# USTC-Computer-Vision/tracking

Measured on AMD Instinct MI355X. Metric: MixtureOfGaussianV2BGS throughput (Mpixels/s; concurrent 1080p30 streams in streams_1080p30), higher is better.
Workload: dtype f32

## Files before the change

tracking_amd/csrc/engine_mog2.h:

```cpp

int mog2_check(bgs_algo, const bgs_params& p) {
  if (p.mog2_nmixtures != bgs::kMog2K) return fail(BGS_ERR_UNSUPPORTED, "MOG2 kernel is built for K=%d mixtures, got %d", bgs::kMog2K, p.mog2_nmixtures);
  return BGS_OK;
}

int mog2_check_geometry(bgs_algo, int, int, int ch) {
  if (ch != 3) return fail(BGS_ERR_UNSUPPORTED, "MixtureOfGaussianV2BGS needs 3 channels: getBackgroundImage asserts nchannels == 3 (MixtureOfGaussianV2BGS.cpp:59)");
  return BGS_OK;
}

struct Mog2State : FamilyState {
  DevPtr<uint8_t> model;
  int sparse_now = 2;
  int sparse_want = 2;
  unsigned launches = 0;
  unsigned confirmed4 = 0;
  unsigned every_left = 0;
  unsigned filter_launches = 0;
  DevPtr<unsigned> d_stat;
  static constexpr int kStatSlots = 8;
  unsigned* h_stat = nullptr;
  hipEvent_t stat_ev[kStatSlots] = {nullptr};
  bool stat_posted[kStatSlots] = {false};
  unsigned stat_seq = 0;
  ~Mog2State() override {
    model.reset(), d_stat.reset();
    if (h_stat) (void)hipHostFree(h_stat);
    for (hipEvent_t ev : stat_ev)
      if (ev) (void)hipEventDestroy(ev);
  }
};
Mog2State& mog2_of(const bgs_engine* e) { return state_of<Mog2State>(e); }

void mog2_stat_read(Mog2State& st) {
  int slot = -1;
  for (unsigned back = 1; back <= (unsigned)Mog2State::kStatSlots && back <= st.stat_seq; ++back) {
    const int i = (int)((st.stat_seq - back) % Mog2State::kStatSlots);
    if (!st.stat_posted[i]) break;
    if (slot < 0 && hipEventQuery(st.stat_ev[i]) == hipSuccess) slot = i;
    if (slot >= 0) st.stat_posted[i] = false;
  }
  if (slot < 0) return;
  const unsigned* hs = st.h_stat + 3 * slot;
  const unsigned total = hs[0], live = hs[1], need = hs[2];
  if (total < 64 * 5) return;
  const float lf = (float)live / (float)total, nf = (float)need / (float)total;
  const int want = (nf < 0.5f * lf && lf - nf > 0.1f) ? 4 : lf < 0.7f ? 2 : 1;
  const bool clear = (want == 4 && nf < 0.35f * lf) || (want != 4 && st.sparse_now == 4 && nf > 0.8f * lf);
  static const bool debug = getenv("BGS_DEBUG_STAT") != nullptr;
  if (debug)
    fprintf(stderr, "[bgs] mog2 auto: %u record slots sampled, %.3f live, %.3f needed after the summaries -> mode %d (now %d)\n", total, lf, nf, want, st.sparse_now);
  const bool confirms = want == 4 && st.sparse_now == 4;
  if (want != st.sparse_now && (clear || want == st.sparse_want)) st.sparse_now = want;
  st.sparse_want = want;
  if (confirms) {
    st.confirmed4++;
  } else {
    st.confirmed4 = 0;
    st.every_left = 8;
  }
}
void mog2_stat_post(Mog2State& st, hipStream_t s) {
  const int i = (int)(st.stat_seq % Mog2State::kStatSlots);
  (void)hipMemcpyAsync(st.h_stat + 3 * i, st.d_stat, 3 * sizeof(unsigned), hipMemcpyDeviceToHost, s);
  (void)hipMemsetAsync(st.d_stat, 0, 3 * sizeof(unsigned), s);
  (void)hipEventRecord(st.stat_ev[i], s);
  st.stat_posted[i] = true;
  st.stat_seq++;
}

int launch_mog2(bgs_engine* e, bgs::Mog2Args& a, hipStream_t s, bool timed = true) {
  const bgs_params& p = e->p;
  a.shadow = p.mog2_detect_shadows && (!p.enable_threshold || ((p.mog2_shadow_value > p.threshold) != (255 > p.threshold)));
  a.want_bg = a.bgimg != nullptr, a.packed = a.fg_bits != nullptr;
  a.xcd_swizzle = e->knob.xcd_swizzle, a.complete = e->knob.mog2_complete;
  Mog2State& st = mog2_of(e);
  const bool autom = timed && e->knob.mog2_sparse == 3;
  if (autom) mog2_stat_read(st);
  int mode = e->knob.mog2_sparse == 3 ? st.sparse_now : e->knob.mog2_sparse;
  const bool every_mean = a.shadow || a.want_bg;
  if (mode >= 4 && every_mean) mode = 2;
  bool sample = false;
  if (autom && mode != 4) {
    const unsigned n = st.launches++;
    if ((n & (n < 64 ? 3u : 15u)) == 0) sample = true, mode = every_mean ? 2 : 4;
  } else if (autom) {
    if (st.every_left > 0 || st.confirmed4 < 2) {
      sample = true;
      if (st.every_left > 0) st.every_left--;
    } else {
      sample = (st.filter_launches++ & 7u) == 0;
    }
  }
  if (mode >= 4 && every_mean) return fail(BGS_ERR_INVALID, "MOG2: the filter kernel cannot deliver the shadow test or the background image");
  a.sparse = mode;
  a.stat = sample ? st.d_stat.p : nullptr;
  if (a.packed && a.npix % 64) return fail(BGS_ERR_UNSUPPORTED, "packed mask needs pixels %% 64 == 0");
  Timed t(e, s, "mog2_update_kernel", timed);
  const dim3 grid(blocks_for(a.npix)), block(bgs::kBlock);
  unsigned every = 1;
  while (grid.x / every > 256) every <<= 1;
  a.stat_mask = every - 1;
  if (mode >= 4)
    hipLaunchKernelGGL((bgs::mog2_update_kernel<bgs::kMog2Filter>), grid, block, 0, s, a);
  else if (mode >= 2)
    hipLaunchKernelGGL((bgs::mog2_update_kernel<bgs::kMog2Count>), grid, block, 0, s, a);
  else
    hipLaunchKernelGGL((bgs::mog2_update_kernel<bgs::kMog2Eager>), grid, block, 0, s, a);
  if (a.stat) mog2_stat_post(st, s);
  return BGS_OK;
}

void mog2_fill_args(const bgs_engine* e, bgs::Mog2Args& m, double lr) {
  const bgs_params& p = e->p;
  m.state = mog2_of(e).model;
  m.alphaT = (float)lr, m.alpha1 = 1.f - m.alphaT, m.prune = (float)(-lr * (double)p.mog2_ct);
  m.Tb = p.mog2_var_threshold, m.TB = p.mog2_background_ratio, m.Tg = p.mog2_var_threshold_gen;
  m.s_min = bgs::mog2_smin(bgs::mog2_tq(m.Tb > m.Tg ? m.Tb : m.Tg));
  m.varInit = p.mog2_var_init, m.varMin = p.mog2_var_min, m.varMax = p.mog2_var_max, m.tau = p.mog2_tau;
  m.thr = p.threshold, m.enable_thr = p.enable_threshold, m.shadow_val = p.mog2_shadow_value;
}

void mog2_clear(bgs_engine* e, const bgs::Mog2Args& m, hipStream_t s) {
  hipLaunchKernelGGL(bgs::mog2_clear_kernel, dim3(blocks_for(m.npix)), dim3(bgs::kBlock), 0, s, m);
}

int launch_mog2_clip(bgs_engine* e, bgs::Mog2ClipArgs& c, int fuse, hipStream_t s) {
  const bgs_params& p = e->p;
  bgs::Mog2Args& a = c.m;
  a.shadow = p.mog2_detect_shadows && (!p.enable_threshold || ((p.mog2_shadow_value > p.threshold) != (255 > p.threshold)));
  a.want_bg = a.bgimg != nullptr, a.packed = a.fg_bits != nullptr;
  a.xcd_swizzle = e->knob.xcd_swizzle, a.complete = e->knob.mog2_complete;
  a.sparse = e->knob.mog2_sparse == 0 ? 0 : 1;
  a.stat = nullptr;
  if (a.packed && a.npix % 64) return fail(BGS_ERR_UNSUPPORTED, "packed mask needs pixels %% 64 == 0");
  Timed t(e, s, "mog2_clip_kernel");
  const dim3 grid(blocks_for(a.npix)), block(bgs::kBlock);
  unsigned every = 1;
  while (grid.x / every > 256) every <<= 1;
  a.stat_mask = every - 1;
#define MOG2_CLIP_CASE(TV) \
  if (fuse == TV) hipLaunchKernelGGL((bgs::mog2_clip_kernel<TV>), grid, block, 0, s, c);
  MOG2_CLIP_CASE(2) MOG2_CLIP_CASE(4) MOG2_CLIP_CASE(8)
#undef MOG2_CLIP_CASE
  return BGS_OK;
}

size_t mog2_state_bytes(const bgs_engine* e) {
  const size_t P = e->n * e->S;
  return (P + bgs::kMog2Tile - 1) / bgs::kMog2Tile * bgs::kMog2TileBytes;
}

int mog2_allocate(bgs_engine* e) {
  Mog2State& st = make_state<Mog2State>(e);
  HIP_TRY(hipMalloc((void**)&st.d_stat.p, 3 * sizeof(unsigned)));
  HIP_TRY(hipMemsetAsync(st.d_stat, 0, 3 * sizeof(unsigned), e->stream()));
  HIP_TRY(hipHostMalloc((void**)&st.h_stat, 3 * Mog2State::kStatSlots * sizeof(unsigned), hipHostMallocDefault));
  for (hipEvent_t& ev : st.stat_ev) HIP_TRY(hipEventCreateWithFlags(&ev, hipEventDisableTiming));
  return model_allocate(e, st.model, mog2_state_bytes(e));
}

uint64_t mog2_key(const bgs_engine* e, int i) { return mog_lr_key(e, i, e->p.mog2_history, 2); }

int mog2_run(bgs_engine* e, int first, int count, const uint8_t* d_frames, uint8_t* d_fg, uint8_t* d_bg, uint64_t* d_bits, hipStream_t s, uint32_t* flags) {
  const bgs_params& p = e->p;
  double lr = p.alpha;
  int64_t nframes = e->seen[first];
  bgs::Mog2Args m{};
  m.state_off = e->n * first, m.npix = e->n * count;
  mog2_fill_args(e, m, 0.0);
  if (nframes == 0 || lr >= 1) {
    mog2_clear(e, m, s);
    nframes = 0;
  }
  ++nframes;
  const int64_t n2 = 2 * nframes;
  lr = (lr >= 0 && nframes > 1) ? lr : 1. / (double)std::min<int64_t>(n2, p.mog2_history);
  mog2_fill_args(e, m, lr);
  m.frame = d_frames, m.fg = d_fg, m.bgimg = d_bg, m.fg_bits = d_bits;
  int rc = launch_mog2(e, m, s);
  if (rc) return rc;
  if (nframes == 1)
    for (int i = first; i < first + count; ++i) e->seen[i] = 0;
  *flags = BGS_FG_VALID | BGS_BG_VALID;
  return BGS_OK;
}

int mog2_clip_fused(bgs_engine* e, int first, int count, int fuse, size_t slab, const uint8_t* fr, uint8_t* fg, uint8_t* bg, uint64_t* bits, hipStream_t s, uint32_t* flags) {
  const bgs_params& p = e->p;
  const int64_t seen = e->seen[first];
  bgs::Mog2ClipArgs c{};
  c.m.state_off = e->n * first, c.m.npix = e->n * count;
  mog2_fill_args(e, c.m, 0.0);
  if (seen == 0) mog2_clear(e, c.m, s);
  for (int j = 0; j < fuse; ++j) {
    const int64_t nf = seen + j + 1;
    const double lr = (p.alpha >= 0 && nf > 1) ? p.alpha : 1. / (double)std::min<int64_t>(2 * nf, p.mog2_history);
    c.alphaT[j] = (float)lr, c.alpha1[j] = 1.f - c.alphaT[j], c.prune[j] = (float)(-lr * (double)p.mog2_ct);
  }
  c.m.frame = fr, c.m.fg = fg, c.m.bgimg = bg, c.m.fg_bits = bits;
  c.frame_stride = slab * 3, c.fg_stride = slab, c.bg_stride = slab * 3, c.bits_stride = slab / 64;
  *flags = BGS_FG_VALID | BGS_BG_VALID;
  return launch_mog2_clip(e, c, fuse, s);
}

int64_t mog2_get_state(bgs_engine* e, int stream, const char* plane, void* dst, size_t cap) {
  const size_t n = e->n, off = n * stream;
  int p0 = -1, np = 0;
  if (!strcmp(plane, "w")) p0 = 0, np = 5;
  if (!strcmp(plane, "var")) p0 = 5, np = 5;
  if (!strcmp(plane, "mu")) p0 = 10, np = 15;
  if (!strcmp(plane, "summary")) p0 = 100, np = 5;
  const bool nm = !strcmp(plane, "nmodes") || !strcmp(plane, "summary_valid");
  const bool want_valid = !strcmp(plane, "summary_valid");
  if (p0 < 0 && !nm) return unknown_plane(e, plane);
  const size_t need = nm ? n : (size_t)np * n * 4;
  if (cap < need) return too_small(plane);
  const size_t T = bgs::kMog2Tile, TB = bgs::kMog2TileBytes;
  const size_t t0 = off / T, t1 = (off + n + T - 1) / T;
  std::vector<uint8_t> tiles((t1 - t0) * TB);
  if (fetch(tiles.data(), mog2_of(e).model + t0 * TB, tiles.size())) return BGS_ERR_HIP;
  for (size_t i = 0; i < n; ++i) {
    const size_t sp = off + i, in = sp % T;
    const uint8_t* tb = tiles.data() + (sp / T - t0) * TB;
    const float* w = reinterpret_cast<const float*>(tb) + in;
    const float* rec = reinterpret_cast<const float*>(tb + bgs::kMog2RecOff) + in * 4;
    const uint16_t* sum = reinterpret_cast<const uint16_t*>(tb + bgs::kMog2SumOff) + in;
    const unsigned meta = reinterpret_cast<const uint16_t*>(tb + bgs::kMog2MetaOff)[in];
    if (nm) {
      ((uint8_t*)dst)[i] = want_valid ? (uint8_t)((meta >> 15) & 1u) : (uint8_t)bgs::mog2_meta_count(meta);
      continue;
    }
    for (int r = 0; r < bgs::kMog2K; ++r) {
      const unsigned f = (meta >> (3 * r)) & 7u;
      const float* rc = f ? rec + (size_t)(f - 1) * T * 4 : nullptr;
      if (p0 == 100) ((uint32_t*)dst)[(size_t)r * n + i] = f ? sum[(size_t)(f - 1) * T] : 0u;
      if (p0 == 0) ((float*)dst)[(size_t)r * n + i] = f ? w[(size_t)r * T] : 0.f;
      if (p0 == 5) ((float*)dst)[(size_t)r * n + i] = f ? rc[0] : 0.f;
      if (p0 == 10)
        for (int c = 0; c < 3; ++c) ((float*)dst)[((size_t)r * 3 + c) * n + i] = f ? rc[1 + c] : 0.f;
    }
  }
  return (int64_t)need;
}

constexpr Family kMog2 = [] {
  Family f{};
  f.check = mog2_check, f.check_geometry = mog2_check_geometry, f.allocate = mog2_allocate, f.key = mog2_key, f.run = mog2_run;
  f.get_state = mog2_get_state, f.clip_fused = mog2_clip_fused, f.clip_fusable = mog_clip_fusable;
  return f;
}();
```

tracking_amd/csrc/kernel_mog2.h:

```cpp
#pragma once
#include "bgs_device.h"

namespace bgs {

constexpr int kMog2K = 5;
constexpr int kMog2Tile = 256;
constexpr size_t kMog2TileBytes = (size_t)kMog2Tile * (4 * kMog2K + 2 * kMog2K + 16 * kMog2K + 2);
constexpr size_t kMog2SumOff = (size_t)kMog2Tile * 4 * kMog2K;
constexpr size_t kMog2RecOff = kMog2SumOff + (size_t)kMog2Tile * 2 * kMog2K;
constexpr size_t kMog2MetaOff = kMog2RecOff + (size_t)kMog2Tile * 16 * kMog2K;
static_assert(kMog2Tile % 64 == 0, "a wave that starts on a multiple of 64 pixels stays inside one tile, any other touches at most two");

struct Mog2Args {
  const uint8_t* frame;
  uint8_t* fg;
  uint8_t* bgimg;
  uint64_t* fg_bits;
  uint8_t* state;
  size_t state_off;
  size_t npix;
  float alphaT, alpha1, prune;
  float Tb, TB, Tg, varInit, varMin, varMax, tau;
  int thr, enable_thr, shadow_val;
  int shadow, want_bg, packed;
  unsigned* stat;
  unsigned stat_mask;
  int sparse;
  int complete;
  int xcd_swizzle;
  uint32_t s_min;
};

struct Mog2Ptr {
  float* w;
  uint16_t* sum;
  float4* rec;
  uint16_t* meta;
};
__device__ __forceinline__ Mog2Ptr mog2_ptr(uint8_t* state, size_t sp) {
  uint8_t* tb = state + (sp / kMog2Tile) * kMog2TileBytes;
  const size_t in = sp % kMog2Tile;
  Mog2Ptr p;
  p.w = reinterpret_cast<float*>(tb) + in;
  p.sum = reinterpret_cast<uint16_t*>(tb + kMog2SumOff) + in;
  p.rec = reinterpret_cast<float4*>(tb + kMog2RecOff) + in;
  p.meta = reinterpret_cast<uint16_t*>(tb + kMog2MetaOff) + in;
  return p;
}
__device__ __forceinline__ size_t mog2_uniform(size_t v) {
  asm("" : "+s"(v));
  return v;
}
struct Mog2Lane {
  uint8_t* state;
  size_t bw, bs, br, bm;
  uint32_t o4, o2, o16;
  static constexpr int kMid = 2 * 4 * kMog2Tile;
  __device__ __forceinline__ float* w(int r) const { return reinterpret_cast<float*>(state + bw + (size_t)o4 + (r * 4 * kMog2Tile - kMid)); }
  __device__ __forceinline__ uint16_t* sum(int s) const { return reinterpret_cast<uint16_t*>(state + bs + (size_t)o2 + s * 2 * kMog2Tile); }
  __device__ __forceinline__ float4* rec(int s) const { return reinterpret_cast<float4*>(state + mog2_uniform(br + (size_t)s * 16 * kMog2Tile) + (size_t)o16); }
  __device__ __forceinline__ float* w_of(uint32_t r) const { return reinterpret_cast<float*>(state + mog2_uniform(bw - kMid) + (size_t)(o4 + r * (4u * kMog2Tile))); }
  __device__ __forceinline__ float4* rec_of(uint32_t s) const { return reinterpret_cast<float4*>(state + br + (size_t)(o16 + s * (16u * kMog2Tile))); }
  __device__ __forceinline__ uint16_t* meta() const { return reinterpret_cast<uint16_t*>(state + bm + (size_t)o2); }
};
__device__ __forceinline__ Mog2Lane mog2_lane(uint8_t* state, size_t first, uint32_t lane) {
  Mog2Lane l;
  const size_t tb = (first / kMog2Tile) * kMog2TileBytes;
  l.state = state;
  l.bw = mog2_uniform(tb + Mog2Lane::kMid), l.bs = mog2_uniform(tb + kMog2SumOff), l.br = mog2_uniform(tb + kMog2RecOff), l.bm = mog2_uniform(tb + kMog2MetaOff);
  const uint32_t in0 = (uint32_t)(first % kMog2Tile);
  uint32_t in = in0 + lane, skip = 0;
  if (in0 + (kWave - 1) >= (uint32_t)kMog2Tile) {
    const bool next = in >= (uint32_t)kMog2Tile;
    in = next ? in - kMog2Tile : in;
    skip = next ? (uint32_t)kMog2TileBytes : 0u;
  }
  l.o4 = in * 4 + skip, l.o2 = in * 2 + skip, l.o16 = in * 16 + skip;
  return l;
}
__device__ __host__ __forceinline__ int mog2_meta_count(unsigned meta) {
  unsigned t = (meta | (meta >> 1) | (meta >> 2)) & 0x1249u;
#ifdef __HIP_DEVICE_COMPILE__
  return __popc(t);
#else
  t = (t & 1u) + ((t >> 3) & 1u) + ((t >> 6) & 1u) + ((t >> 9) & 1u) + ((t >> 12) & 1u);
  return (int)t;
#endif
}

constexpr float kMog2SumVar = 32.f, kMog2SumVarTight = 24.f;
__device__ __host__ __forceinline__ uint32_t mog2_summary(float var, float m0, float m1, float m2) {
  const bool inside = m0 >= 0.f && m0 < 256.f && m1 >= 0.f && m1 < 256.f && m2 >= 0.f && m2 < 256.f;
  const uint32_t cls = (inside && var <= kMog2SumVarTight) ? 0u : 1u;
  const uint32_t q0 = inside ? (uint32_t)(int)m0 >> 3 : 0u, q1 = inside ? (uint32_t)(int)m1 >> 3 : 0u, q2 = inside ? (uint32_t)(int)m2 >> 3 : 0u;
  return q0 | (q1 << 5) | (q2 << 10) | (cls << 15);
}
__device__ __host__ __forceinline__ bool mog2_summary_ok(uint32_t word, float var, float m0, float m1, float m2) {
  const float b0 = (float)((word & 0x1fu) << 3), b1 = (float)(((word >> 5) & 0x1fu) << 3), b2 = (float)(((word >> 10) & 0x1fu) << 3);
  const float e0 = m0 - b0, e1 = m1 - b1, e2 = m2 - b2;
  const bool means = (e0 >= -2.f && e0 <= 9.f) && (e1 >= -2.f && e1 <= 9.f) && (e2 >= -2.f && e2 <= 9.f);
  const bool tightable = var <= kMog2SumVarTight && m0 >= 0.f && m0 < 256.f && m1 >= 0.f && m1 < 256.f && m2 >= 0.f && m2 < 256.f;
  return (word >> 15) ? !tightable : (means && var <= kMog2SumVar);
}
__device__ __host__ __forceinline__ uint32_t mog2_tq(float Tmax) {
  const float c = 3.f * kMog2SumVar * Tmax;
  return c < 1.0e9f ? (uint32_t)(int)c + 4u : 0xffffffffu;
}
constexpr uint32_t kMog2SMax = 93u, kMog2SNever = 0xffffffffu;
__device__ __host__ __forceinline__ uint32_t mog2_smin(uint32_t tq) {
  for (uint32_t S = 4u; S <= kMog2SMax; ++S) {
    const uint32_t B = 8u * S - 28u;
    if (B * B > tq) return S;
  }
  return kMog2SNever;
}
__device__ __host__ __forceinline__ uint32_t mog2_pixq(uint32_t pix) { return (pix >> 3) & 0x1f1f1fu; }
__device__ __host__ __forceinline__ uint32_t mog2_spread(uint32_t word) { return (word & 0x1fu) | ((word << 3) & 0x1f00u) | ((word << 6) & 0x1f0000u); }
__device__ __host__ __forceinline__ bool mog2_reject_s(uint32_t word, uint32_t S, uint32_t s_min) { return !(word >> 15) & (S >= s_min); }
__device__ __forceinline__ bool mog2_reject(uint32_t word, uint32_t pixq, uint32_t s_min) {
  return mog2_reject_s(word, __builtin_amdgcn_sad_u8(pixq, mog2_spread(word), 0u), s_min);
}

enum { kMog2Stream = 0, kMog2BySlot = 1, kMog2Ranked = 2, kMog2One = 3 };
struct Mog2Px {
  float w[kMog2K];
  int sl[kMog2K];
};
struct Mog2Recs {
  float4 rc[kMog2K];
  int k0, cnt;
  unsigned cm, bgm, mm;
};

template <int ORD>
__device__ __forceinline__ void mog2_swap(Mog2Px& s, Mog2Recs& R, int i, int j) {
  const float t = s.w[i];
  s.w[i] = s.w[j], s.w[j] = t;
  const int u = s.sl[i];
  s.sl[i] = s.sl[j], s.sl[j] = u;
  if constexpr (ORD == kMog2Ranked) {
    const float4 c = R.rc[i];
    R.rc[i] = R.rc[j], R.rc[j] = c;
  }
}

template <int ORD>
__device__ __forceinline__ float4 mog2_pick(const Mog2Recs& R, int code) {
  static_assert(ORD == kMog2BySlot, "ranked records are indexed by rank; the filter kernel holds one record or none");
  float4 v = make_float4(0.f, 0.f, 0.f, 0.f);
#pragma unroll
  for (int j = 0; j < kMog2K; ++j) {
    const bool here = code == j + 1;
    const float4 c = R.rc[j];
    v.x = here ? c.x : v.x, v.y = here ? c.y : v.y, v.z = here ? c.z : v.z, v.w = here ? c.w : v.w;
  }
  return v;
}
template <int ORD>
__device__ __forceinline__ float4 mog2_rec_at(const Mog2Px& s, const Mog2Recs& R, int mode) {
  if constexpr (ORD == kMog2Ranked)
    return R.rc[mode];
  else
    return mog2_pick<ORD>(R, s.sl[mode]);
}
template <int ORD>
__device__ __forceinline__ float4 mog2_pick_now(const Mog2Recs& R, int code, int hit, float4 out) {
  const float4 v = mog2_pick<ORD>(R, code);
  const bool h = code == hit;
  return make_float4(h ? out.x : v.x, h ? out.y : v.y, h ? out.z : v.z, h ? out.w : v.w);
}

template <int ORD>
__device__ __forceinline__ float4 mog2_rec_now(const Mog2Px& s, const Mog2Recs& R, int mode, int hit, float4 out) {
  if constexpr (ORD == kMog2Ranked)
    return R.rc[mode];
  else
    return mog2_pick_now<ORD>(R, s.sl[mode], hit, out);
}

template <int ORD>
__device__ __forceinline__ bool mog2_shadow(const Mog2Px& s, const Mog2Recs& R, int hit, float4 out, int nmodes, float x0, float x1, float x2, const Mog2Args& a) {
  bool done = false, result = false;
  float tWeight = 0.f;
#pragma unroll
  for (int mode = 0; mode < kMog2K; ++mode) {
    if (mode < nmodes && !done) {
      const float4 v = mog2_rec_now<ORD>(s, R, mode, hit, out);
      float num = 0.0f, den = 0.0f;
      num += x0 * v.y;
      den += v.y * v.y;
      num += x1 * v.z;
      den += v.z * v.z;
      num += x2 * v.w;
      den += v.w * v.w;
      if (den == 0) {
        done = true;
      } else {
        if (num <= den && num >= a.tau * den) {
          const float q = div_rn(num, den);
          float d2a = 0.0f, dD;
          dD = q * v.y - x0, d2a += dD * dD;
          dD = q * v.z - x1, d2a += dD * dD;
          dD = q * v.w - x2, d2a += dD * dD;
          if (d2a < a.Tb * v.x * q * q) result = true, done = true;
        }
        if (!done) {
          tWeight += s.w[mode];
          if (tWeight > a.TB) done = true;
        }
      }
    }
  }
  return result;
}

template <int ORD>
__device__ __forceinline__ int mog2_pixel(Mog2Px& s, Mog2Recs& R, int& nmodes_io, float x0, float x1, float x2, const Mog2Args& a, int& hit, float4& out,
                                          const float alphaT, const float alpha1, const float prune, const unsigned rej) {
  bool background = false, fitsPDF = false;
  int nmodes = nmodes_io;
  const int nNewModes = nmodes;
  float totalWeight = 0.f;
  hit = 0;
  out = make_float4(0.f, 0.f, 0.f, 0.f);
#pragma unroll
  for (int mode = 0; mode < kMog2K; ++mode) {
    if (mode < nmodes) {
      float weight = alpha1 * s.w[mode] + prune;
      bool matched = false;
      if (!fitsPDF && !((rej >> s.sl[mode]) & 1u)) {
        const float4 v = mog2_rec_at<ORD>(s, R, mode);
        const float var = v.x;
        const float d0 = v.y - x0, d1 = v.z - x1, d2 = v.w - x2;
        const float dist2 = d0 * d0 + d1 * d1 + d2 * d2;
        if (totalWeight < a.TB && dist2 < a.Tb * var) background = true;
        if (dist2 < a.Tg * var) {
          fitsPDF = true;
          matched = true;
          weight += alphaT;
          const float k = div_rn(alphaT, weight);
          float varnew = var + k * (dist2 - var);
          varnew = varnew > a.varMin ? varnew : a.varMin;
          varnew = varnew < a.varMax ? varnew : a.varMax;
          out = make_float4(varnew, v.y - k * d0, v.z - k * d1, v.w - k * d2);
          hit = s.sl[mode];
          if constexpr (ORD == kMog2Ranked) R.rc[mode] = out;
        }
      }
      const bool pruned = weight < -prune;
      if (pruned) nmodes--;
      s.w[mode] = pruned ? 0.f : weight;
      if (matched) {
        bool moving = true;
#pragma unroll
        for (int i = mode; i > 0; --i) {
          moving = moving && !(weight < s.w[i - 1]);
          if (moving) mog2_swap<ORD>(s, R, i, i - 1);
        }
      }
      totalWeight += pruned ? 0.f : weight;
    }
  }
  totalWeight = div_rn(1.f, totalWeight);
#pragma unroll
  for (int mode = 0; mode < kMog2K; ++mode)
    if (mode < nmodes) s.w[mode] *= totalWeight;
  nmodes = nNewModes;
  if (!fitsPDF) {
    const int slot = (nmodes == kMog2K) ? s.sl[kMog2K - 1] : nmodes + 1;
    const int mode = (nmodes == kMog2K) ? kMog2K - 1 : nmodes++;
#pragma unroll
    for (int k = 0; k < kMog2K; ++k) {
      if (k == mode) {
        s.w[k] = (nmodes == 1) ? 1.f : alphaT;
        s.sl[k] = slot;
        if constexpr (ORD == kMog2Ranked) R.rc[k] = make_float4(a.varInit, x0, x1, x2);
      } else if (nmodes != 1 && k < nmodes - 1) {
        s.w[k] *= alpha1;
      }
    }
    out = make_float4(a.varInit, x0, x1, x2);
    hit = slot;
    bool moving = true;
#pragma unroll
    for (int i = kMog2K - 1; i > 0; --i) {
      if (i <= nmodes - 1) {
        moving = moving && !(alphaT < s.w[i - 1]);
        if (moving) mog2_swap<ORD>(s, R, i, i - 1);
      }
    }
  }
  nmodes_io = nmodes;
  if (background) return 0;
  if (a.shadow) {
    if (mog2_shadow<ORD>(s, R, hit, out, nmodes, x0, x1, x2, a)) return a.shadow_val;
  }
  return 255;
}

template <int ORD, bool FEAT>
__device__ __forceinline__ int mog2_pixel_lockstep(Mog2Px& s, const Mog2Recs& R, const Mog2Lane& mp, const int wave_cand, int& nmodes_io, float x0, float x1,
                                                   float x2, const Mog2Args& a, int& hit, float4& out, const float alphaT, const float alpha1, const float prune) {
  static_assert(ORD != kMog2Ranked, "records by slot, streamed, or the single one");
  static_assert(!FEAT || ORD == kMog2BySlot, "the shadow test needs every record in registers");
  bool background = false, fitsPDF = false;
  int nmodes = nmodes_io;
  const int nNewModes = nmodes;
  float totalWeight = 0.f;
  hit = 0;
  out = make_float4(0.f, 0.f, 0.f, 0.f);
  unsigned cm = 0, bgm = 0, mm = 0;
  bool c1 = false, b1 = false, m1 = false;
  int k1 = 0;
  if constexpr (ORD == kMog2One) {
    const float4 v = R.rc[0];
    const float d0 = v.y - x0, d1 = v.z - x1, d2 = v.w - x2;
    const float dist2 = d0 * d0 + d1 * d1 + d2 * d2;
    c1 = R.cnt > 0, k1 = R.k0 + 1;
    b1 = dist2 < a.Tb * v.x, m1 = dist2 < a.Tg * v.x;
  } else if constexpr (ORD == kMog2Stream) {
    cm = R.cm, bgm = R.bgm, mm = R.mm;
  } else {
#pragma unroll
    for (int j = 0; j < kMog2K; ++j) {
      if (j < wave_cand) {
        const float4 v = R.rc[j];
        const float d0 = v.y - x0, d1 = v.z - x1, d2 = v.w - x2;
        const float dist2 = d0 * d0 + d1 * d1 + d2 * d2;
        const int code = j + 1;
        const bool is = j < R.cnt;
        cm |= (unsigned)is << code;
        bgm |= (unsigned)(is && dist2 < a.Tb * v.x) << code;
        mm |= (unsigned)(is && dist2 < a.Tg * v.x) << code;
      }
    }
  }
  float wmatch = 0.f;
  int rstar = 0;
#pragma unroll
  for (int mode = 0; mode < kMog2K; ++mode) {
    if (mode < nmodes) {
      float weight = alpha1 * s.w[mode] + prune;
      const int code = s.sl[mode];
      const bool c = ORD == kMog2One ? (c1 && code == k1) : (bool)((cm >> code) & 1u);
      if (!fitsPDF && c) {
        const bool b = ORD == kMog2One ? b1 : (bool)((bgm >> code) & 1u);
        const bool m = ORD == kMog2One ? m1 : (bool)((mm >> code) & 1u);
        if (totalWeight < a.TB && b) background = true;
        if (m) {
          fitsPDF = true;
          weight += alphaT;
          wmatch = weight, rstar = mode, hit = code;
        }
      }
      const bool pruned = weight < -prune;
      if (pruned) nmodes--;
      s.w[mode] = pruned ? 0.f : weight;
      totalWeight += pruned ? 0.f : weight;
    }
  }
  if (fitsPDF) {
    float4 v;
    if constexpr (ORD == kMog2Stream)
      v = *mp.rec_of((uint32_t)(hit - 1));
    else if constexpr (ORD == kMog2One)
      v = R.rc[0];
    else
      v = wave_cand == 1 ? R.rc[0] : mog2_pick<ORD>(R, hit);
    const float var = v.x;
    const float d0 = v.y - x0, d1 = v.z - x1, d2 = v.w - x2;
    const float dist2 = d0 * d0 + d1 * d1 + d2 * d2;
    const float k = div_rn(alphaT, wmatch);
    float varnew = var + k * (dist2 - var);
    varnew = varnew > a.varMin ? varnew : a.varMin;
    varnew = varnew < a.varMax ? varnew : a.varMax;
    out = make_float4(varnew, v.y - k * d0, v.z - k * d1, v.w - k * d2);
    bool moving = true;
#pragma unroll
    for (int i = kMog2K - 1; i > 0; --i) {
      const bool in = i <= rstar;
      moving = in ? (moving & !(wmatch < s.w[i - 1])) : moving;
      const bool sw = in & moving;
      const float wi = s.w[i], wj = s.w[i - 1];
      s.w[i] = sw ? wj : wi, s.w[i - 1] = sw ? wi : wj;
      const int ci = s.sl[i], cj = s.sl[i - 1];
      s.sl[i] = sw ? cj : ci, s.sl[i - 1] = sw ? ci : cj;
    }
  }
  totalWeight = div_rn(1.f, totalWeight);
#pragma unroll
  for (int mode = 0; mode < kMog2K; ++mode)
    if (mode < nmodes) s.w[mode] *= totalWeight;
  nmodes = nNewModes;
  if (!fitsPDF) {
    const int slot = (nmodes == kMog2K) ? s.sl[kMog2K - 1] : nmodes + 1;
    const int mode = (nmodes == kMog2K) ? kMog2K - 1 : nmodes++;
#pragma unroll
    for (int k = 0; k < kMog2K; ++k) {
      if (k == mode) {
        s.w[k] = (nmodes == 1) ? 1.f : alphaT;
        s.sl[k] = slot;
      } else if (nmodes != 1 && k < nmodes - 1) {
        s.w[k] *= alpha1;
      }
    }
    out = make_float4(a.varInit, x0, x1, x2);
    hit = slot;
    bool moving = true;
    Mog2Recs none;
#pragma unroll
    for (int i = kMog2K - 1; i > 0; --i) {
      if (i <= nmodes - 1) {
        moving = moving && !(alphaT < s.w[i - 1]);
        if (moving) mog2_swap<ORD>(s, none, i, i - 1);
      }
    }
  }
  nmodes_io = nmodes;
  if (background) return 0;
  if constexpr (FEAT) {
    if (a.shadow) {
      if (mog2_shadow<ORD>(s, R, hit, out, nmodes, x0, x1, x2, a)) return a.shadow_val;
    }
  }
  return 255;
}

template <int ORD>
__device__ __forceinline__ void mog2_background(const Mog2Px& s, const Mog2Recs& R, int hit, float4 out, int nmodes, float TB, int& b0, int& b1, int& b2) {
  float v0 = 0.f, v1 = 0.f, v2 = 0.f, totalWeight = 0.f;
  bool stop = false;
#pragma unroll
  for (int g = 0; g < kMog2K; ++g) {
    if (g < nmodes && !stop) {
      const float4 v = mog2_rec_now<ORD>(s, R, g, hit, out);
      const float w = s.w[g];
      v0 += w * v.y;
      v1 += w * v.z;
      v2 += w * v.w;
      totalWeight += w;
      if (totalWeight > TB) stop = true;
    }
  }
  const float inv = div_rn(1.f, totalWeight);
  b0 = sat_u8(v0 * inv), b1 = sat_u8(v1 * inv), b2 = sat_u8(v2 * inv);
}

__device__ __forceinline__ void mog2_group_or(unsigned v, unsigned& or2, unsigned& or8, unsigned& or16) {
  v |= (unsigned)__builtin_amdgcn_mov_dpp((int)v, 0xB1, 0xf, 0xf, true);
  or2 = v;
  v |= (unsigned)__builtin_amdgcn_mov_dpp((int)v, 0x4E, 0xf, 0xf, true);
  v |= (unsigned)__builtin_amdgcn_mov_dpp((int)v, 0x141, 0xf, 0xf, true);
  or8 = v;
  v |= (unsigned)__builtin_amdgcn_mov_dpp((int)v, 0x140, 0xf, 0xf, true);
  or16 = v;
}

__device__ __forceinline__ void mog2_stream(const Mog2Lane& mp, Mog2Recs& R, const unsigned need, const bool valid_in, const bool sampled, const uint32_t pix,
                                            const Mog2Args& a, uint32_t (&sm)[kMog2K], int& would) {
  const float x0 = (float)(pix & 0xffu), x1 = (float)((pix >> 8) & 0xffu), x2 = (float)(pix >> 16);
  const uint32_t pixq = mog2_pixq(pix), k_first = (uint32_t)R.k0;
  const bool rebuild = __any(!valid_in);
  unsigned cm = 0, bgm = 0, mm = 0;
  int fresh = 0;
  float4 cur = *mp.rec_of((need & 1u) ? 0u : k_first);
#pragma unroll
  for (int k = 0; k < kMog2K; ++k) {
    float4 nxt = cur;
    if (k + 1 < kMog2K) nxt = *mp.rec_of(((need >> (k + 1)) & 1u) ? (uint32_t)(k + 1) : k_first);
    const bool is = (need >> k) & 1u;
    const float d0 = cur.y - x0, d1 = cur.z - x1, d2 = cur.w - x2;
    const float dist2 = d0 * d0 + d1 * d1 + d2 * d2;
    cm |= (unsigned)is << (k + 1);
    bgm |= (unsigned)(is && dist2 < a.Tb * cur.x) << (k + 1);
    mm |= (unsigned)(is && dist2 < a.Tg * cur.x) << (k + 1);
    if (rebuild) {
      const uint32_t word = mog2_summary(cur.x, cur.y, cur.z, cur.w);
      const bool mine = is && !valid_in;
      sm[k] = mine ? word : sm[k];
      if (sampled) fresh += (int)(mine && !mog2_reject(word, pixq, a.s_min));
    }
    cur = nxt;
  }
  R.cm = cm, R.bgm = bgm, R.mm = mm;
  would = valid_in ? would : fresh;
}

__device__ __forceinline__ void mog2_stat_add(const Mog2Args& a, const uint32_t lane, const int nm_in, const int would) {
  unsigned s_live = 0, s_need = 0;
#pragma unroll
  for (int bit = 0; bit < 3; ++bit) {
    s_live += (unsigned)__popcll(__ballot((nm_in >> bit) & 1)) << bit;
    s_need += (unsigned)__popcll(__ballot((would >> bit) & 1)) << bit;
  }
  const unsigned lanes = (unsigned)__popcll(__ballot(1));
  if (lane == 0) {
    atomicAdd(a.stat, lanes * kMog2K);
    atomicAdd(a.stat + 1, s_live);
    atomicAdd(a.stat + 2, s_need);
  }
}

constexpr int kMog2ClipMax = 8;
struct Mog2ClipArgs {
  Mog2Args m;
  size_t frame_stride;
  size_t fg_stride, bg_stride, bits_stride;
  float alphaT[kMog2ClipMax], alpha1[kMog2ClipMax], prune[kMog2ClipMax];
};

enum { kMog2Eager = 1, kMog2Count = 2, kMog2Filter = 4 };

template <int MODE, int T>
__device__ __forceinline__ void mog2_body(const Mog2Args& a, const size_t frame_stride, const size_t fg_stride, const size_t bg_stride, const size_t bits_stride,
                                          const float* alphaT, const float* alpha1, const float* prune) {
  static_assert(T == 1 || MODE == kMog2Eager, "clip launches load eagerly");
  constexpr int ORD = MODE == kMog2Filter ? kMog2Stream : T > 1 ? kMog2Ranked : kMog2BySlot;
  constexpr bool FEAT = MODE != kMog2Filter;
  size_t blk = blockIdx.x;
  if (a.xcd_swizzle) {
    const size_t per = gridDim.x >> 3, main = per << 3;
    if (blk < main) blk = (blk & 7) * per + (blk >> 3);
  }
  const uint32_t lane = threadIdx.x & (kWave - 1);
  const size_t pw = blk * kBlock + (uint32_t)__builtin_amdgcn_readfirstlane((int)(threadIdx.x & ~(uint32_t)(kWave - 1)));
  if (pw >= a.npix) return;
  const size_t left = a.npix - pw;
  if (lane >= (left < (size_t)kWave ? (uint32_t)left : (uint32_t)kWave)) return;
  uint32_t pix[T];
  const uint8_t* const fw = a.frame + pw * 3;
#pragma unroll
  for (int t = 0; t < T; ++t) {
    const uint8_t* f = fw + (size_t)t * frame_stride + lane * 3u;
    pix[t] = (uint32_t)f[0] | ((uint32_t)f[1] << 8) | ((uint32_t)f[2] << 16);
  }
  const Mog2Lane mp = mog2_lane(a.state, a.state_off + pw, lane);
  const unsigned meta_raw = *mp.meta();
  const unsigned meta_in = meta_raw & 0x7fffu;
  const bool valid_in = (meta_raw >> 15) & 1u;
  const int nm_in = mog2_meta_count(meta_in);
  const bool dense = MODE == kMog2Eager && a.sparse == 0;
  const bool sampled = MODE != kMog2Eager && a.stat && (blockIdx.x & a.stat_mask) == 0;
  float wv[kMog2K];
  uint32_t sm[kMog2K];
  Mog2Recs R;
  R.cnt = kMog2K;
  int wave_cand = kMog2K;
#pragma unroll
  for (int k = 0; k < kMog2K; ++k) sm[k] = 0u;
  if constexpr (MODE == kMog2Eager) {
#pragma unroll
    for (int k = 0; k < kMog2K; ++k) {
      wv[k] = *mp.w(k);
      R.rc[k] = *mp.rec(k);
      if (dense) sm[k] = *mp.sum(k);
    }
  } else if constexpr (MODE == kMog2Count) {
    wv[0] = *mp.w(0);
    R.rc[0] = *mp.rec(0);
    int wave_nm = 0;
#pragma unroll
    for (int n = 1; n <= kMog2K; ++n)
      if (__any(nm_in >= n)) wave_nm = n;
    wave_cand = wave_nm <= 2 ? 2 : wave_nm;
    if (wave_nm <= 2) {
      const uint32_t idx = 1 < nm_in ? 1u : 0u;
      wv[1] = *mp.w_of(idx), R.rc[1] = *mp.rec_of(idx);
#pragma unroll
      for (int k = 2; k < kMog2K; ++k) wv[k] = 0.f, R.rc[k] = make_float4(0.f, 0.f, 0.f, 0.f);
    } else {
#pragma unroll
      for (int k = 1; k < kMog2K; ++k) {
        const uint32_t idx = k < nm_in ? (uint32_t)k : 0u;
        wv[k] = *mp.w_of(idx), R.rc[k] = *mp.rec_of(idx);
      }
    }
#pragma unroll
    for (int k = 0; k < kMog2K; ++k) wv[k] = k < nm_in ? wv[k] : 0.f;
    R.cnt = nm_in;
  } else {
#pragma unroll
    for (int k = 0; k < kMog2K; ++k) wv[k] = *mp.w(k), sm[k] = *mp.sum(k);
    const uint32_t pixq = mog2_pixq(pix[0]);
    unsigned need = 0;
#pragma unroll
    for (int k = 0; k < kMog2K; ++k) {
      const bool live = k < nm_in;
      const bool r = (live & valid_in) & mog2_reject(sm[k], pixq, a.s_min);
      need |= (unsigned)(live && !r) << k;
    }
    R.cnt = __popc(need);
    R.k0 = (int)min((unsigned)__builtin_ctzg(need, 32), (unsigned)(kMog2K - 1));
    int would = R.cnt;
    if (!__any(R.cnt > 1)) {
      wave_cand = 1;
      R.rc[0] = *mp.rec_of((uint32_t)R.k0);
      if (sampled && !valid_in) {
        const float4 c = R.rc[0];
        would = (int)(R.cnt > 0 && !mog2_reject(mog2_summary(c.x, c.y, c.z, c.w), pixq, a.s_min));
      }
    } else {
      mog2_stream(mp, R, need, valid_in, sampled, pix[0], a, sm, would);
    }
    if (sampled) mog2_stat_add(a, lane, nm_in, would);
  }
  if constexpr (MODE == kMog2Count) {
    if (sampled) mog2_stat_add(a, lane, nm_in, nm_in);
  }
  Mog2Px s;
#pragma unroll
  for (int r = 0; r < kMog2K; ++r) s.sl[r] = (int)((meta_in >> (3 * r)) & 7u), s.w[r] = wv[r];
  if constexpr (ORD == kMog2Ranked) {
    Mog2Recs Q;
#pragma unroll
    for (int r = 0; r < kMog2K; ++r) Q.rc[r] = mog2_pick<kMog2BySlot>(R, s.sl[r]);
#pragma unroll
    for (int r = 0; r < kMog2K; ++r) R.rc[r] = Q.rc[r];
  }
  unsigned dirty = 0;
  const bool one = MODE == kMog2Filter && wave_cand == 1;
  int nm = nm_in, hit = 0;
  float4 out = make_float4(0.f, 0.f, 0.f, 0.f);
#pragma unroll
  for (int t = 0; t < T; ++t) {
    const float x0 = (float)(pix[t] & 0xffu), x1 = (float)((pix[t] >> 8) & 0xffu), x2 = (float)(pix[t] >> 16);
    int raw;
    if constexpr (ORD == kMog2Ranked)
      raw = mog2_pixel<ORD>(s, R, nm, x0, x1, x2, a, hit, out, alphaT[t], alpha1[t], prune[t], 0u);
    else if (one)
      raw = mog2_pixel_lockstep<kMog2One, false>(s, R, mp, 1, nm, x0, x1, x2, a, hit, out, alphaT[t], alpha1[t], prune[t]);
    else
      raw = mog2_pixel_lockstep<ORD, FEAT>(s, R, mp, wave_cand, nm, x0, x1, x2, a, hit, out, alphaT[t], alpha1[t], prune[t]);
    const int m = thr_bin(raw, a.thr, a.enable_thr);
    if (a.fg) (a.fg + pw + (size_t)t * fg_stride)[lane] = (uint8_t)m;
    if (a.packed) {
      const uint64_t word = __ballot(m != 0);
      if (lane == 0) (a.fg_bits + (pw >> 6) + (size_t)t * bits_stride)[0] = word;
    }
    if constexpr (FEAT) {
      if (a.want_bg) {
        int b0, b1, b2;
        mog2_background<ORD>(s, R, hit, out, nm, a.TB, b0, b1, b2);
        uint8_t* o = a.bgimg + pw * 3 + (size_t)t * bg_stride + lane * 3u;
        o[0] = (uint8_t)b0, o[1] = (uint8_t)b1, o[2] = (uint8_t)b2;
      }
    }
    dirty |= 1u << hit;
  }
  unsigned d = 0;
#pragma unroll
  for (int r = 0; r < kMog2K; ++r) d |= (unsigned)(s.w[r] != wv[r]) << r;
  d |= (dirty >> 1) << 6;
  bool valid_out = false;
  if constexpr (MODE == kMog2Filter) {
    uint32_t old = 0;
#pragma unroll
    for (int q = 0; q < kMog2K; ++q) old = hit == q + 1 ? sm[q] : old;
    const bool keep = valid_in && hit <= nm_in && mog2_summary_ok(old, out.x, out.y, out.z, out.w);
    if (__any(!keep)) {
#pragma unroll
      for (int q = 0; q < kMog2K; ++q) {
        const bool changed = hit == q + 1;
        if ((changed && !keep) || (!valid_in && q < nm)) {
          if (one) {
            const float4 c = R.rc[0];
            sm[q] = mog2_summary(changed ? out.x : c.x, changed ? out.y : c.y, changed ? out.z : c.z, changed ? out.w : c.w);
          } else {
            sm[q] = changed ? mog2_summary(out.x, out.y, out.z, out.w) : sm[q];
          }
          d |= 1u << (11 + q);
        }
      }
    }
    valid_out = true;
  }
  unsigned meta_out = valid_out ? 0x8000u : 0u;
#pragma unroll
  for (int r = 0; r < kMog2K; ++r) meta_out |= (unsigned)s.sl[r] << (3 * r);
  d |= (unsigned)(meta_out != meta_raw) << 5;
  if (dense) {
    d = 0xffffu;
  } else if (a.complete) {
    unsigned d2, d8, d16;
    mog2_group_or(d, d2, d8, d16);
    unsigned c = (d8 & 0x1fu) | (d16 & 0x20u);
    if constexpr (MODE == kMog2Filter) c |= d16 & 0xf800u;
    if constexpr (MODE == kMog2Eager) c |= d2 & 0x7c0u;
    d |= c;
  }
#pragma unroll
  for (int r = 0; r < kMog2K; ++r)
    if ((d >> r) & 1u) *mp.w(r) = s.w[r];
  if ((d >> 5) & 1u) *mp.meta() = (uint16_t)meta_out;
  if constexpr (MODE == kMog2Eager) {
#pragma unroll
    for (int q = 0; q < kMog2K; ++q) {
      if ((d >> (11 + q)) & 1u) *mp.sum(q) = (uint16_t)sm[q];
      if ((d >> (6 + q)) & 1u) {
        float4 v;
        if constexpr (T == 1) {
          const bool h = hit == q + 1;
          v = make_float4(h ? out.x : R.rc[q].x, h ? out.y : R.rc[q].y, h ? out.z : R.rc[q].z, h ? out.w : R.rc[q].w);
        } else {
          v = make_float4(0.f, 0.f, 0.f, 0.f);
#pragma unroll
          for (int r = 0; r < kMog2K; ++r) {
            const bool h = s.sl[r] == q + 1;
            v.x = h ? R.rc[r].x : v.x, v.y = h ? R.rc[r].y : v.y, v.z = h ? R.rc[r].z : v.z, v.w = h ? R.rc[r].w : v.w;
          }
        }
        *mp.rec(q) = v;
      }
    }
  } else {
    *mp.rec_of((uint32_t)(hit - 1)) = out;
    if constexpr (MODE == kMog2Filter) {
#pragma unroll
      for (int q = 0; q < kMog2K; ++q)
        if ((d >> (11 + q)) & 1u) *mp.sum(q) = (uint16_t)sm[q];
    }
  }
}

template <int MODE>
__global__ __launch_bounds__(kBlock) void mog2_update_kernel(const Mog2Args a) {
  mog2_body<MODE, 1>(a, 0, 0, 0, 0, &a.alphaT, &a.alpha1, &a.prune);
}
#ifndef BGS_MOG2_FILTER_WAVES
#define BGS_MOG2_FILTER_WAVES 6
#endif
template <>
__global__ __launch_bounds__(kBlock) __attribute__((amdgpu_waves_per_eu(1, BGS_MOG2_FILTER_WAVES))) void mog2_update_kernel<kMog2Filter>(const Mog2Args a) {
  mog2_body<kMog2Filter, 1>(a, 0, 0, 0, 0, &a.alphaT, &a.alpha1, &a.prune);
}

template <int T>
__global__ __launch_bounds__(kBlock) void mog2_clip_kernel(const Mog2ClipArgs c) {
  mog2_body<kMog2Eager, T>(c.m, c.frame_stride, c.fg_stride, c.bg_stride, c.bits_stride, c.alphaT, c.alpha1, c.prune);
}

__global__ __launch_bounds__(kBlock) void mog2_clear_kernel(const Mog2Args a) {
  const size_t p = (size_t)blockIdx.x * kBlock + threadIdx.x;
  if (p >= a.npix) return;
  const Mog2Ptr mp = mog2_ptr(a.state, a.state_off + p);
#pragma unroll
  for (int k = 0; k < kMog2K; ++k) {
    mp.w[(size_t)k * kMog2Tile] = 0.f;
    mp.sum[(size_t)k * kMog2Tile] = 0;
    mp.rec[(size_t)k * kMog2Tile] = make_float4(0.f, 0.f, 0.f, 0.f);
  }
  *mp.meta = 0;
}

}
```

Baseline: 72540.

## Skip loading trailing mixture records when the lead Gaussian matches in count mode

In the count-mode MOG2 kernel, each pixel first tests whether its top-ranked mixture matches. When it does (and neither shadows nor the background image are needed), only the weights of the other modes are loaded and their mean/variance records are skipped, wave-uniformly when every lane agrees. Sampled launches now always use count mode and record both the summary-filter statistic and a new loaded-record count in a fourth stat word. A debug plane exposes these counters. The aim is less model-state memory traffic, at the cost of an extra distance test and a wave-wide vote per pixel.

```diff
diff --git a/tracking_amd/csrc/engine_mog2.h b/tracking_amd/csrc/engine_mog2.h
--- a/tracking_amd/csrc/engine_mog2.h
+++ b/tracking_amd/csrc/engine_mog2.h
@@ -19,6 +19,7 @@
   unsigned filter_launches = 0;
   DevPtr<unsigned> d_stat;
   static constexpr int kStatSlots = 8;
+  static constexpr int kStatWords = 4;
   unsigned* h_stat = nullptr;
   hipEvent_t stat_ev[kStatSlots] = {nullptr};
   bool stat_posted[kStatSlots] = {false};
@@ -41,7 +42,7 @@
     if (slot >= 0) st.stat_posted[i] = false;
   }
   if (slot < 0) return;
-  const unsigned* hs = st.h_stat + 3 * slot;
+  const unsigned* hs = st.h_stat + Mog2State::kStatWords * slot;
   const unsigned total = hs[0], live = hs[1], need = hs[2];
   if (total < 64 * 5) return;
   const float lf = (float)live / (float)total, nf = (float)need / (float)total;
@@ -62,8 +63,8 @@
 }
 void mog2_stat_post(Mog2State& st, hipStream_t s) {
   const int i = (int)(st.stat_seq % Mog2State::kStatSlots);
-  (void)hipMemcpyAsync(st.h_stat + 3 * i, st.d_stat, 3 * sizeof(unsigned), hipMemcpyDeviceToHost, s);
-  (void)hipMemsetAsync(st.d_stat, 0, 3 * sizeof(unsigned), s);
+  (void)hipMemcpyAsync(st.h_stat + Mog2State::kStatWords * i, st.d_stat, Mog2State::kStatWords * sizeof(unsigned), hipMemcpyDeviceToHost, s);
+  (void)hipMemsetAsync(st.d_stat, 0, Mog2State::kStatWords * sizeof(unsigned), s);
   (void)hipEventRecord(st.stat_ev[i], s);
   st.stat_posted[i] = true;
   st.stat_seq++;
@@ -83,7 +84,7 @@
   bool sample = false;
   if (autom && mode != 4) {
     const unsigned n = st.launches++;
-    if ((n & (n < 64 ? 3u : 15u)) == 0) sample = true, mode = every_mean ? 2 : 4;
+    if ((n & (n < 64 ? 3u : 15u)) == 0) sample = true, mode = 2;
   } else if (autom) {
     if (st.every_left > 0 || st.confirmed4 < 2) {
       sample = true;
@@ -153,9 +154,10 @@
 
 int mog2_allocate(bgs_engine* e) {
   Mog2State& st = make_state<Mog2State>(e);
-  HIP_TRY(hipMalloc((void**)&st.d_stat.p, 3 * sizeof(unsigned)));
-  HIP_TRY(hipMemsetAsync(st.d_stat, 0, 3 * sizeof(unsigned), e->stream()));
-  HIP_TRY(hipHostMalloc((void**)&st.h_stat, 3 * Mog2State::kStatSlots * sizeof(unsigned), hipHostMallocDefault));
+  HIP_TRY(hipMalloc((void**)&st.d_stat.p, Mog2State::kStatWords * sizeof(unsigned)));
+  HIP_TRY(hipMemsetAsync(st.d_stat, 0, Mog2State::kStatWords * sizeof(unsigned), e->stream()));
+  HIP_TRY(hipHostMalloc((void**)&st.h_stat, Mog2State::kStatWords * Mog2State::kStatSlots * sizeof(unsigned), hipHostMallocDefault));
+  std::memset(st.h_stat, 0, Mog2State::kStatWords * Mog2State::kStatSlots * sizeof(unsigned));
   for (hipEvent_t& ev : st.stat_ev) HIP_TRY(hipEventCreateWithFlags(&ev, hipEventDisableTiming));
   return model_allocate(e, st.model, mog2_state_bytes(e));
 }
@@ -205,6 +207,17 @@
 }
 
 int64_t mog2_get_state(bgs_engine* e, int stream, const char* plane, void* dst, size_t cap) {
+  if (!strcmp(plane, "mog2_auto")) {
+    const Mog2State& st = mog2_of(e);
+    unsigned rec[Mog2State::kStatWords] = {0};
+    for (unsigned back = 1; back <= (unsigned)Mog2State::kStatSlots && back <= st.stat_seq; ++back) {
+      const int i = (int)((st.stat_seq - back) % Mog2State::kStatSlots);
+      if (hipEventQuery(st.stat_ev[i]) != hipSuccess) continue;
+      std::memcpy(rec, st.h_stat + Mog2State::kStatWords * i, sizeof(rec));
+      break;
+    }
+    return copy_host(plane, dst, cap, rec, sizeof(rec));
+  }
   const size_t n = e->n, off = n * stream;
   int p0 = -1, np = 0;
   if (!strcmp(plane, "w")) p0 = 0, np = 5;
diff --git a/tracking_amd/csrc/kernel_mog2.h b/tracking_amd/csrc/kernel_mog2.h
--- a/tracking_amd/csrc/kernel_mog2.h
+++ b/tracking_amd/csrc/kernel_mog2.h
@@ -501,6 +501,17 @@
   }
 }
 
+__device__ __forceinline__ void mog2_stat_add_loaded(const Mog2Args& a, const uint32_t lane, const int loaded) {
+  unsigned s_loaded = 0;
+#pragma unroll
+  for (int bit = 0; bit < 3; ++bit) s_loaded += (unsigned)__popcll(__ballot((loaded >> bit) & 1)) << bit;
+  if (lane == 0) atomicAdd(a.stat + 3, s_loaded);
+}
+
+#ifndef BGS_MOG2_WEIGHTS_ONLY
+#define BGS_MOG2_WEIGHTS_ONLY 1
+#endif
+
 constexpr int kMog2ClipMax = 8;
 struct Mog2ClipArgs {
   Mog2Args m;
@@ -558,26 +569,57 @@
   } else if constexpr (MODE == kMog2Count) {
     wv[0] = *mp.w(0);
     R.rc[0] = *mp.rec(0);
-    int wave_nm = 0;
-#pragma unroll
-    for (int n = 1; n <= kMog2K; ++n)
+    bool lead_match;
+    {
+      const float x0 = (float)(pix[0] & 0xffu), x1 = (float)((pix[0] >> 8) & 0xffu), x2 = (float)(pix[0] >> 16);
+      const float4 v = R.rc[0];
+      const float d0 = v.y - x0, d1 = v.z - x1, d2 = v.w - x2;
+      const float dist2 = d0 * d0 + d1 * d1 + d2 * d2;
+      lead_match = (meta_in & 7u) == 1u && dist2 < a.Tg * v.x;
+    }
+    const bool rule = lead_match && !(a.shadow || a.want_bg);
+    const bool first = rule && !sampled;
+    R.cnt = first ? 1 : nm_in;
+    int wave_nm = 0, wave_cnt = 0;
+#pragma unroll
+    for (int n = 1; n <= kMog2K; ++n) {
       if (__any(nm_in >= n)) wave_nm = n;
-    wave_cand = wave_nm <= 2 ? 2 : wave_nm;
-    if (wave_nm <= 2) {
+      if (__any(R.cnt >= n)) wave_cnt = n;
+    }
+    if (BGS_MOG2_WEIGHTS_ONLY && wave_cnt <= 1) {
+      wave_cand = 1;
+#pragma unroll
+      for (int k = 1; k < kMog2K; ++k) {
+        wv[k] = *mp.w_of(k < nm_in ? (uint32_t)k : 0u);
+        R.rc[k] = make_float4(0.f, 0.f, 0.f, 0.f);
+      }
+    } else if (wave_nm <= 2) {
+      wave_cand = 2;
       const uint32_t idx = 1 < nm_in ? 1u : 0u;
-      wv[1] = *mp.w_of(idx), R.rc[1] = *mp.rec_of(idx);
+      wv[1] = *mp.w_of(idx), R.rc[1] = *mp.rec_of(first ? 0u : idx);
 #pragma unroll
       for (int k = 2; k < kMog2K; ++k) wv[k] = 0.f, R.rc[k] = make_float4(0.f, 0.f, 0.f, 0.f);
     } else {
+      wave_cand = wave_cnt < 2 ? 2 : wave_cnt;
 #pragma unroll
       for (int k = 1; k < kMog2K; ++k) {
         const uint32_t idx = k < nm_in ? (uint32_t)k : 0u;
-        wv[k] = *mp.w_of(idx), R.rc[k] = *mp.rec_of(idx);
+        wv[k] = *mp.w_of(idx), R.rc[k] = *mp.rec_of(first ? 0u : idx);
       }
     }
 #pragma unroll
     for (int k = 0; k < kMog2K; ++k) wv[k] = k < nm_in ? wv[k] : 0.f;
-    R.cnt = nm_in;
+    if (sampled) {
+      const uint32_t pixq = mog2_pixq(pix[0]);
+      int would = 0;
+#pragma unroll
+      for (int k = 0; k < kMog2K; ++k) {
+        const float4 c = R.rc[k];
+        would += (int)(k < nm_in && !mog2_reject(mog2_summary(c.x, c.y, c.z, c.w), pixq, a.s_min));
+      }
+      mog2_stat_add(a, lane, nm_in, would);
+      mog2_stat_add_loaded(a, lane, rule ? 1 : nm_in);
+    }
   } else {
 #pragma unroll
     for (int k = 0; k < kMog2K; ++k) wv[k] = *mp.w(k), sm[k] = *mp.sum(k);
@@ -603,9 +645,6 @@
       mog2_stream(mp, R, need, valid_in, sampled, pix[0], a, sm, would);
     }
     if (sampled) mog2_stat_add(a, lane, nm_in, would);
-  }
-  if constexpr (MODE == kMog2Count) {
-    if (sampled) mog2_stat_add(a, lane, nm_in, nm_in);
   }
   Mog2Px s;
 #pragma unroll
```

New measurement: 72260. No clear change (-0.4%).
